# advimman/lama

Hardware: AMD Instinct MI355X
Metric: inpainted images/sec at 512x512 big-lama (higher is better)
Workload: dtype f32 (3-term f16 split on the 16-bit MFMA, fp32 accumulate, fp32 activations); 1 GPU; big-lama FFCResNetGenerator 512x512 batch=8/GPU fp32 (BASELINE configs[1]), mask-compose + generator + blend + u8, random-init weights; global_batch=8, resolution=512, parallelism=dp1, hip_graph=True, precision=f16x3, split_batch=1, full=False

## Files before the change

include/lama_hip.h:

```cpp
#ifndef LAMA_HIP_H
#define LAMA_HIP_H
#include <stddef.h>
#include <stdint.h>

#ifdef __cplusplus
extern "C" {
#endif

#define LAMA_HIP_VERSION 112

#define LAMA_OK 0
#define LAMA_ERR_BAD_ARG (-1)
#define LAMA_ERR_UNSUPPORTED (-2)
#define LAMA_ERR_WORKSPACE (-3)

#define LAMA_ACT_NONE 0
#define LAMA_ACT_RELU 1
#define LAMA_ACT_SIGMOID 2
#define LAMA_ACT_TANH 3

#define LAMA_PAD_ZERO 0
#define LAMA_PAD_REFLECT 1

#define LAMA_PREC_F32 0
// ... 116 lines not shown
    int32_t up_mg[4];
    int32_t* head_list;
    int32_t* head_count;
    int32_t* up_list[4];
    int32_t* up_count[4];
} lama_tail_lists;
size_t lama_tail_lists_workspace_bytes(int32_t batch, int32_t H, int32_t W, const lama_tail_lists* lists);
int lama_tail_lists_build(void* stream, const lama_tensor* mask, int32_t batch, const lama_tail_lists* lists, void* workspace, size_t workspace_bytes);
int lama_conv2d_list_fwd(void* stream, const lama_conv2d_args* args, const int32_t* list, const int32_t* count, int32_t head_rs);
int32_t lama_conv2d_list_supported(const lama_conv2d_args* args, int32_t head_rs);

#define LAMA_CONV_FAMILY_F32 0
#define LAMA_CONV_FAMILY_GEMM1X1_WK 1
#define LAMA_CONV_FAMILY_GEMM1X1_W4 2
#define LAMA_CONV_FAMILY_GEMM1X1_WS 3
#define LAMA_CONV_FAMILY_CONV_WR 4
#define LAMA_CONV_FAMILY_CONVT2 5
#define LAMA_CONV_FAMILY_STEM7 6
#define LAMA_CONV_FAMILY_HEAD7 7
#define LAMA_CONV_FAMILY_LDS 8
#define LAMA_CONV_GEO_WR(wmv, kg, ksc1, twlog, s2, coop, roll, fuse1, xs, ys) \
    ((wmv) | (kg) << 4 | (ksc1) << 8 | (twlog) << 12 | (s2) << 16 | (coop) << 17 | (roll) << 18 | (fuse1) << 19 | (xs) << 20 | (ys) << 21)
int lama_conv2d_route_query(const lama_conv2d_args* args, int32_t head_rs, int32_t* family, int32_t* geometry);

int lama_affine_act_fwd(void* stream, const lama_tensor* x, const float* scale, const float* shift, int32_t act,
                        const lama_tensor* y, int32_t batch);
int lama_reflect_pad_fwd(void* stream, const lama_tensor* x, int32_t pad, const lama_tensor* y, int32_t batch);

int lama_act_bwd(void* stream, const lama_tensor* g, const lama_tensor* y, int32_t act, const lama_tensor* gout, int32_t batch);
int lama_add_fwd(void* stream, const lama_tensor* a, const lama_tensor* b, const lama_tensor* out, int32_t batch);
int lama_reflect_pad_bwd(void* stream, const lama_tensor* gp, const lama_tensor* addend, int32_t pad, const lama_tensor* g,
                         int32_t batch);
int lama_reflect_pad_bwd_fused(void* stream, const lama_tensor* gp, const lama_tensor* add1, const lama_tensor* add2, int32_t pad,
                               const lama_tensor* mask_y, int32_t act, const lama_tensor* g, const lama_tensor* gm, int32_t batch,
                               const float* ring);
size_t lama_dgrad_ring_bytes(int32_t batch, int32_t cout, int32_t H, int32_t W);
int lama_dgrad_ring_fwd(void* stream, const lama_tensor* g, const float* w_ring, int32_t cout, float* ring, int32_t batch);
int lama_gauss5_fwd(void* stream, const lama_tensor* x, const lama_tensor* y, int32_t batch);
int lama_gauss5_bwd(void* stream, const lama_tensor* gy, const lama_tensor* gx, int32_t batch);
int lama_bilinear_fwd(void* stream, const lama_tensor* x, const lama_tensor* y, int32_t batch);
int lama_bilinear_bwd(void* stream, const lama_tensor* gy, const lama_tensor* gx, int32_t batch);
int lama_threshold_fwd(void* stream, const lama_tensor* x, float thr, const lama_tensor* y, int32_t batch);
int lama_erode_fwd(void* stream, const lama_tensor* x, const float* se, int32_t kh, int32_t kw, float max_val, const lama_tensor* y,
                   int32_t batch);
int lama_l1_masked_fwd(void* stream, const lama_tensor* pred, const lama_tensor* target, const lama_tensor* mask, float thr,
                       int32_t select_ge, double* accum, int32_t batch);
// ... 70 lines not shown
```

lama_amd/_lib.py:

```python
from __future__ import annotations

import ctypes as C
import os
from typing import Optional

import torch

ACT_NONE, ACT_RELU, ACT_SIGMOID, ACT_TANH = 0, 1, 2, 3
PAD_ZERO, PAD_REFLECT = 0, 1
PREC_F32, PREC_BF16X3, PREC_F16X3, PREC_F16 = 0, 1, 2, 3
CONV_COOPERATIVE = 1
CONV_DEFER_OUT = 2
CONV_SIBLINGS_SHIFT = 8
DT_F32, DT_F16, DT_SPLIT16 = 0, 1, 2
(CONV_FAM_F32, CONV_FAM_GEMM1X1_WK, CONV_FAM_GEMM1X1_W4, CONV_FAM_GEMM1X1_WS, CONV_FAM_CONV_WR, CONV_FAM_CONVT2, CONV_FAM_STEM7, CONV_FAM_HEAD7,
 CONV_FAM_LDS) = range(9)


def conv_geo_wr(wmv, kg, ksc1, twlog, s2=0, coop=0, roll=0, fuse1=0, xs=0, ys=0) -> int:
    return wmv | kg << 4 | ksc1 << 8 | twlog << 12 | s2 << 16 | coop << 17 | roll << 18 | fuse1 << 19 | xs << 20 | ys << 21


def conv_geo_lds(bm, bn, mode=0, trf=0) -> int:
    return bm | bn << 8 | mode << 20 | trf << 22
POOL_MAX, POOL_AVG_EXCLUDE_PAD = 0, 1
ABI_VERSION = 112
PREC_NAMES = {'f32': PREC_F32, 'bf16x3': PREC_BF16X3, 'f16x3': PREC_F16X3, 'f16': PREC_F16}

_DEFAULT = os.path.join(os.path.dirname(os.path.abspath(__file__)), 'lib', 'liblama_hip.so')


class LamaError(RuntimeError):

    def __init__(self, msg: str = '', code=None):
        super().__init__(msg)
        self.code = code


class LamaRangeError(LamaError):
# ... 79 lines not shown
    def __init__(self, path: Optional[str] = None, host_emulated: bool = False):
        self.host_emulated = host_emulated
        path = path or _DEFAULT
        if not os.path.exists(path):
            raise LamaError(f'{path} not found: build it with `python -m lama_amd.build` '
                            f'(hipcc --offload-arch=gfx950); lama_amd has no fallback path')
        self.path = path
        L = self._l = C.CDLL(path)
        i32, i64, vp, sz = C.c_int32, C.c_int64, C.c_void_p, C.c_size_t
        T = C.POINTER(Tensor4)
        L.lama_version.restype = C.c_int
        L.lama_error_string.restype = C.c_char_p
        L.lama_error_string.argtypes = [C.c_int]
        L.lama_conv2d_packed_weight_bytes.restype = i64
        L.lama_conv2d_packed_weight_bytes.argtypes = [i32] * 7
        L.lama_conv2d_pack_weight.restype = C.c_int
        L.lama_conv2d_pack_weight.argtypes = [vp, vp, vp, i32, i32, i32, i32, i32, i32, i32, vp]
        L.lama_conv2d_fwd.restype = C.c_int
        L.lama_conv2d_fwd.argtypes = [vp, C.POINTER(Conv2dArgs)]
        L.lama_conv2d_list_fwd.restype, L.lama_conv2d_list_fwd.argtypes = C.c_int, [vp, C.POINTER(Conv2dArgs), vp, vp, i32]
        L.lama_conv2d_list_supported.restype, L.lama_conv2d_list_supported.argtypes = i32, [C.POINTER(Conv2dArgs), i32]
        L.lama_conv2d_route_query.restype = C.c_int
        L.lama_conv2d_route_query.argtypes = [C.POINTER(Conv2dArgs), i32, C.POINTER(C.c_int32), C.POINTER(C.c_int32)]
        L.lama_tail_lists_workspace_bytes.restype, L.lama_tail_lists_workspace_bytes.argtypes = sz, [i32, i32, i32, C.POINTER(TailLists)]
        L.lama_tail_lists_build.restype, L.lama_tail_lists_build.argtypes = C.c_int, [vp, T, i32, C.POINTER(TailLists), vp, sz]
        L.lama_rfft2_fwd.restype = C.c_int
        L.lama_rfft2_fwd.argtypes = [vp, T, T, i32, vp, sz]
        L.lama_irfft2_fwd.restype = C.c_int
        L.lama_irfft2_fwd.argtypes = [vp, T, T, T, i32, vp, sz]
        L.lama_winograd_out_fwd.restype = C.c_int
        L.lama_winograd_out_fwd.argtypes = [vp, C.POINTER(Conv2dArgs), vp, sz]
        L.lama_rfft2_winograd_out_fwd.restype = C.c_int
        L.lama_rfft2_winograd_out_fwd.argtypes = [vp, T, T, i32, vp, sz, C.POINTER(Conv2dArgs), vp, sz]
        L.lama_rfft2_masked_fwd.restype = C.c_int
        L.lama_rfft2_masked_fwd.argtypes = [vp, T, T, T, i32, vp, sz]
        L.lama_irfft2_masked_fwd.restype = C.c_int
        L.lama_irfft2_masked_fwd.argtypes = [vp, T, T, T, T, i32, vp, sz]
        L.lama_fft_workspace_bytes.restype = sz
        L.lama_fft_workspace_bytes.argtypes = [i32] * 4
        L.lama_fft_route_query.restype = C.c_int
        L.lama_fft_route_query.argtypes = [T, T, T, T, i32, i32, vp, sz, C.POINTER(C.c_int32), C.POINTER(C.c_int32)]
        L.lama_fourier_unit_workspace_bytes.restype = sz
        L.lama_fourier_unit_workspace_bytes.argtypes = [i32] * 4
        L.lama_fourier_unit_fwd.restype = C.c_int
        L.lama_fourier_unit_fwd.argtypes = [vp, T, vp, vp, T, i32, i32, i32, vp, sz, vp]
        L.lama_fourier_unit_winograd_out_fwd.restype = C.c_int
# ... 94 lines not shown
            cout, cin, kh, kw = w.shape
        nbytes = self._l.lama_conv2d_packed_weight_bytes(cout, cin, kh, kw, stride, int(transposed), precision)
        if nbytes <= 0:
            raise LamaError(f'unsupported conv geometry {tuple(w.shape)} stride={stride} transposed={transposed}')
        if precision in (PREC_F16X3, PREC_F16) and w.numel():
            ws = w if scale is None else w * (scale.float().view(1, -1, 1, 1) if transposed else scale.float().view(-1, 1, 1, 1))
            amax = float(ws.abs().max())
            if not amax <= F16_MAX:
                raise LamaRangeError(f'folded conv weight |w| max {amax:.3g} exceeds the fp16 split range ({F16_MAX}); use bf16x3 or f32')
        dst = torch.empty(nbytes // 4, dtype=torch.float32, device=w.device)
        sc = None if scale is None else scale.contiguous().float()
        self.check(self._l.lama_conv2d_pack_weight(self.stream_of(w), w.data_ptr(), None if sc is None else sc.data_ptr(),
                                                   cout, cin, kh, kw, stride, int(transposed), precision, dst.data_ptr()),
                   'lama_conv2d_pack_weight')
        if w.is_cuda:
            torch.cuda.current_stream(w.device).synchronize()
        return dst

    def conv2d(self, x: Tensor4, w_packed: torch.Tensor, y: Tensor4, batch: int, k: int, stride: int = 1, pad: int = 0,
               pad_mode: int = PAD_REFLECT, transposed: bool = False, bias: Optional[torch.Tensor] = None,
               act: int = ACT_NONE, resid: Optional[Tensor4] = None, x2: Optional[Tensor4] = None,
               w2_packed: Optional[torch.Tensor] = None, precision: int = PREC_F32, stream: int = 0,
               range_flag: Optional[torch.Tensor] = None, fuse1: Optional[tuple] = None, cooperative: bool = False, siblings_log2: int = 0,
               tile_list: Optional[tuple] = None, query: bool = False, route: bool = False):
        a = Conv2dArgs()
        a.x, a.w_packed = x, w_packed.data_ptr()
        a.kh = a.kw = k
        a.stride, a.pad, a.pad_mode, a.transposed = stride, pad, pad_mode, int(transposed)
        if x2 is not None:
            a.x2, a.w2_packed = x2, w2_packed.data_ptr()
        a.bias = None if bias is None else bias.data_ptr()
        a.act = act
        if resid is not None:
            a.resid = resid
        a.y, a.batch, a.precision = y, batch, precision
        a.range_flag = None if range_flag is None else range_flag.data_ptr()
        if fuse1 is not None:
            a.fuse1_w, a.fuse1_bias, a.fuse1_y = fuse1[0].data_ptr(), fuse1[1].data_ptr(), fuse1[2]
        a.flags = (CONV_COOPERATIVE if cooperative else 0) | (int(siblings_log2) << CONV_SIBLINGS_SHIFT)
        if route:
            fam, geo = C.c_int32(-1), C.c_int32(-1)
            rc = self._l.lama_conv2d_route_query(C.byref(a), -1 if tile_list is None else int(tile_list[2]), C.byref(fam), C.byref(geo))
            return (int(rc), fam.value, geo.value) if rc == 0 else (int(rc), None, None)
        if tile_list is not None:
            lst, cnt, head_rs = tile_list
            if query:
                return self._l.lama_conv2d_list_supported(C.byref(a), int(head_rs)) == 1
            self.check(self._l.lama_conv2d_list_fwd(stream, C.byref(a), lst.data_ptr(), cnt.data_ptr(), int(head_rs)), 'lama_conv2d_list_fwd')
            return None
        self.check(self._l.lama_conv2d_fwd(stream, C.byref(a)), 'lama_conv2d_fwd')

    def tail_lists_alloc(self, batch: int, H: int, W: int, head_rs: int, up_mg, device) -> dict:
        n_up = len(up_mg)
        if n_up > 4 or H % (1 << n_up) or W % (1 << n_up) or head_rs < 8 or head_rs % 8:
            raise LamaError(f'tail lists: {n_up} upsamplings of a {H} x {W} plane, head_rs {head_rs}')

        def pair(n):
            return torch.zeros(n, dtype=torch.int32, device=device), torch.zeros(1, dtype=torch.int32, device=device)

        cd = lambda a, b: (a + b - 1) // b
        head = pair(batch * cd(W, 26) * cd(H, head_rs))
        up = [pair(batch * cd(H >> (i + 1), 4) * cd(W >> (i + 1), 32) * int(up_mg[i])) for i in range(n_up)]
        a = TailLists()
        a.n_up, a.head_rs = n_up, head_rs
        a.head_list, a.head_count = head[0].data_ptr(), head[1].data_ptr()
        for i in range(n_up):
# ... 492 lines not shown
```

lama_amd/csrc/conv_mfma.hip:

```cpp
#include "common.h"

typedef float f32x16 __attribute__((ext_vector_type(16)));

#define CONV_BN 128
#define CONV_MAX_TAPS 49

struct ConvSeg {
    const float* x;
    long long bstride;
    int C, H, W;
    const float* w;
    int stride, pad_mode;
    int dy0, dx0;
    int PH, PW;
    int tapoff[CONV_MAX_TAPS];
};

struct ConvParams {
    ConvSeg s1, s2;
    const float* bias;
    const float* resid;
    long long resid_bstride;
    float* y;
    long long y_bstride;
// ... 658 lines not shown
        p.tiles_y = lama_ceil_div(p.GH, CONV_BN >> twlog);
        int T2 = 0, BKC2 = 0;
        if (has2) {
            T2 = 1; BKC2 = pl2.BKC[0];
            if (!fill_seg(&p.s2, a->x2, (const float*)a->w2_packed, pl2, 0, 1, LAMA_PAD_ZERO, twlog, BKC2 * CONV_BN / LAMA_NTHREADS, false))
                return LAMA_ERR_UNSUPPORTED;
        }
        int rc = launch_conv((hipStream_t)stream, p, pl.T[cls], pl.BKC[cls], T2, BKC2, pl.BM, query != nullptr);
        if (rc != LAMA_OK) return rc;
    }
    return LAMA_OK;
}

extern "C" int lama_conv2d_fwd(void* stream, const lama_conv2d_args* a) { return conv2d_impl(stream, a, nullptr); }

extern "C" int lama_conv2d_list_fwd(void* stream, const lama_conv2d_args* a, const int32_t* list, const int32_t* count, int32_t head_rs) {
    if (!list || !count) return LAMA_ERR_BAD_ARG;
    const LamaTileList tl = {list, count, head_rs};
    return conv2d_impl(stream, a, &tl);
}
extern "C" int lama_conv2d_route_query(const lama_conv2d_args* a, int32_t head_rs, int32_t* family, int32_t* geometry) {
    if (!family || !geometry) return LAMA_ERR_BAD_ARG;
    const LamaTileList tl = {nullptr, nullptr, head_rs};
    int32_t q[2] = {0, 0};
    const int rc = conv2d_impl(nullptr, a, head_rs < 0 ? nullptr : &tl, q);
    if (rc == LAMA_OK) { *family = q[0]; *geometry = q[1]; }
    return rc;
}
extern "C" int32_t lama_conv2d_list_supported(const lama_conv2d_args* a, int32_t head_rs) {
    int32_t family, geometry;
    return lama_conv2d_route_query(a, head_rs < 0 ? 0 : head_rs, &family, &geometry) == LAMA_OK ? 1 : 0;
}
```

lama_amd/csrc/conv_split3.inc:

```
#include "common.h"
#include <stdlib.h>

typedef float f32x16 __attribute__((ext_vector_type(16)));
typedef float f32x2 __attribute__((ext_vector_type(2)));
#ifndef CB_HALF
#define CB_HALF 0
#endif
#ifndef CB_HF_W2
#define CB_HF_W2 1
#endif
#if CB_F16
typedef _Float16 cb_half_t;
#define CB_MFMA __builtin_amdgcn_mfma_f32_32x32x16_f16
#if CB_HALF
#define CB_NAME(x) x##_f16
#else
#define CB_NAME(x) x##_f16x3
#endif
#else
typedef __bf16 cb_half_t;
#define CB_MFMA __builtin_amdgcn_mfma_f32_32x32x16_bf16
#define CB_NAME(x) x##_bf16x3
#endif
typedef cb_half_t bf16x2 __attribute__((ext_vector_type(2)));
// ... 897 lines not shown
        pp.kw = kw;
        pp.transposed = transposed;
        for (int t = 0; t < pl.T[cls]; ++t) { pp.tap_ky[t] = pl.ky[cls][t]; pp.tap_kx[t] = pl.kx[cls][t]; }
        long long total = pl.cls_bytes[cls] / 32;
        int grid = (int)((total + 255) / 256);
        if (grid > 4096) grid = 4096;
        hipLaunchKernelGGL(CB_NAME(conv_pack_kernel), dim3(grid), dim3(256), 0, stream, pp);
        LAMA_CHECK_LAUNCH();
    }
    return LAMA_OK;
}

int CB_NAME(lama_cb_conv2d_fwd)(hipStream_t stream, const lama_conv2d_args* a, int Ho, int Wo, const LamaTileList* tl, int32_t* query) {
    CbPlan pl, pl2;
    if (!cb_make_plan(a->y.C, a->x.C, a->kh, a->kw, a->stride, a->pad, a->transposed, &pl)) return LAMA_ERR_UNSUPPORTED;
    const bool has2 = a->x2.ptr != nullptr;
    if (has2 && (!cb_make_plan(a->y.C, a->x2.C, 1, 1, 1, 0, 0, &pl2) || pl.mode)) return LAMA_ERR_UNSUPPORTED;
    int io = (a->x.dtype == LAMA_DT_F16 ? 1 : 0) | (a->y.dtype == LAMA_DT_F16 ? 2 : 0) | ((has2 && a->x2.dtype == LAMA_DT_F16) ? CB_IO_X2H : 0);
    if ((io != CB_IO_F32) != (CB_HALF != 0)) return LAMA_ERR_UNSUPPORTED;
    io |= (a->x.dtype == LAMA_DT_SPLIT16 ? CB_IO_XS : 0) | (a->y.dtype == LAMA_DT_SPLIT16 ? CB_IO_YS : 0);
    const CbPlan* p2 = has2 ? &pl2 : nullptr;
    CbRoute r;
    const int rc = cb_route(a, pl, p2, Ho, Wo, io, tl, &r);
    if (query && rc == LAMA_OK) { query[0] = r.family; query[1] = cb_route_geometry(r); }
    if (query || rc != LAMA_OK) return rc;
    const long long HW = (long long)Ho * Wo;
    switch (r.family) {
        case CB_FAM_WK: return wk_launch(stream, a, pl, HW, r);
        case CB_FAM_W4: return w4_launch(stream, a, pl, HW, r);
        case CB_FAM_WS: return ws_launch(stream, a, pl, HW, r);
        case CB_FAM_WR: return wr_launch(stream, a, pl, p2, Ho, Wo, r);
        case CB_FAM_CT: return ct_launch(stream, a, pl, tl, r);
        case CB_FAM_STEM: return stem_launch(stream, a, pl, Ho, Wo, r);
        case CB_FAM_HEAD: return head_launch(stream, a, pl, Ho, Wo, tl, r);
        case CB_FAM_LDS: {
            CbParams p;
            lds_fill(&p, a, pl, p2, Ho, Wo, r);
            return cb_launch(stream, p, pl.T[0], has2 ? 1 : 0, r.BM, r.maxu, r.trf, r.mode, io, r.grid, r.shmem);
        }
    }
    return CB_ERR_ROUTE;
}

#if !CB_HALF
int CB_NAME(lama_cb_mdconv_fwd)(hipStream_t stream, const lama_conv2d_args* a, int groups, int min_dilation) {
    const int cout = a->y.C, cin = a->x.C, H = a->x.H, W = a->x.W;
    const int dmax = min_dilation << (groups - 1);
// ... 236 lines not shown
```

lama_amd/csrc/conv_wreg_dev.inc:

```

template <int T, int KSC, int WMV, int KG>
struct CwShape {
    static_assert((T == 9 && (KSC == 2 || (KSC == 1 && KG == 1))) || (T == 1 && KSC == 4),
                  "3x3 over 32-channel chunks (16-channel chunks in the 4 x 1 geometry) or 1x1 over 64-channel chunks");
    static_assert(KG == 1 || KG == 2, "K-groups");
    static constexpr int THREADS = 64 * WMV * KG;
    static constexpr int NKG = T * KSC / KG;
    static constexpr int WPS = WMV * KG / 4;
    static constexpr int PFD = (T == 1 && KG == 2) ? 2 : 1;
#ifndef LAMA_CW_RING9
#define LAMA_CW_RING9 0
#endif
    static constexpr int RING = (T == 9) ? ((LAMA_CW_RING9 && KG == 2 && WPS <= 2) ? 9 : ((KSC == 2 && WMV == 4 && KG == 1) ? 6 : 3)) : ((WPS >= 3) ? 2 : 4);
    static constexpr bool BDB = WPS <= 2;
    static constexpr int NOCT = 2 * KSC;
    static_assert((PFD * NKG) % RING == 0, "ring slot must be a compile-time function of the unrolled position");
};

struct CwFrag {
    bf16x8 bh[4], bl[4];
};

template <int T, int KSC, int WMV, int KG, int ABL = 0, int SCH = 2, bool HF = false, bool HI = HF, bool ROLL = false, int NU = 2, bool XS = false>
__device__ __forceinline__ void cw_segment(const CbSeg& s, int F, int b, int gy0, int gx0, int TWlog, char* pbuf0, int pbytes,
// ... 362 lines not shown
    const int tiy = tile % p.tiles_y;
    const int b = tile / p.tiles_y;
    const int TW = 1 << p.TWlog, TH = 128 >> p.TWlog;
    const int gy0 = tiy * TH, gx0 = tix * TW;
    const int tid = threadIdx.x, lane = tid & 63, wave = LAMA_WAVE_UNIFORM(tid >> 6);
    const int kg = wave / WMV, wm = wave % WMV;
    const int F = mt * WMV + wm;
    const int Fc = F < p.s1.mft ? F : p.s1.mft - 1;

    long long* trace = nullptr;
    if constexpr (ABL & 64) {
        trace = p.trace + (long long)blockIdx.x * 32;
        if (threadIdx.x == 0) trace[0] = LAMA_CLOCK();
    }
    f32x16 acc[4];
#pragma unroll
    for (int j = 0; j < 4; ++j)
#pragma unroll
        for (int r = 0; r < 16; ++r) acc[j][r] = 0.0f;

    unsigned rw = 0;
    const int Fw = (ABL & 256) ? Fc % 6 : Fc;
    cw_segment<T1, KSC1, WMV, KG, (ABL & 255), SCH, HF, HI1, ROLL && T1 == 9, NU, XS>(p.s1, Fw, b, gy0, gx0, p.TWlog, lama_smem, p.pbytes, acc, rw, trace);
    if constexpr (T2 > 0) cw_segment<T2, KSC2, WMV, KG, (ABL & 65), SCH, HF, HI2>(p.s2, Fw, b, gy0, gx0, p.TWlog, lama_smem, p.pbytes, acc, rw, (ABL & 64) ? trace + 7 : nullptr);
    cb_range_report(rw, p.range_flag);

    const long long plane = (long long)p.Ho * p.Wo;
    const int khalf4 = 4 * (lane >> 5);
    const int kplane = khalf4 * (int)plane;
    auto row_u = [&](int r) { return F * 32 + (r & 3) + 8 * (r >> 2); };
    float bv[16];
#pragma unroll
    for (int r = 0; r < 16; ++r) bv[r] = p.bias ? p.bias[row_u(r) + khalf4 < p.M ? row_u(r) + khalf4 : p.M - 1] : 0.0f;
    constexpr int NRV = (WMV * KG / 4 >= 3) ? 1 : 2;
    float rv[NRV][16];
    auto frag_off = [&](int j, bool& pv) {
        const int n = j * 32 + (lane & 31);
        const int gy = gy0 + (n >> p.TWlog), gx = gx0 + (n & (TW - 1));
        pv = gy < p.GH && gx < p.GW;
        return (gy < p.GH ? gy : p.GH - 1) * p.Wo + (gx < p.GW ? gx : p.GW - 1);
    };
    auto load_resid = [&](int j, int slot) {
        bool pv;
        const int po = frag_off(j, pv);
#pragma unroll
        for (int r = 0; r < 16; ++r) {
            const int mu = row_u(r), muc = mu < p.M ? mu : p.M - 1;
// ... 191 lines not shown
```

lama_amd/csrc/conv_wreg_host.inc:

```

#define G4_SUP 2
#ifndef GK_DEFAULT_MODE
#define GK_DEFAULT_MODE 1
#endif

enum CbFamily {
    CB_FAM_WK = LAMA_CONV_FAMILY_GEMM1X1_WK, CB_FAM_W4 = LAMA_CONV_FAMILY_GEMM1X1_W4, CB_FAM_WS = LAMA_CONV_FAMILY_GEMM1X1_WS,
    CB_FAM_WR = LAMA_CONV_FAMILY_CONV_WR, CB_FAM_CT = LAMA_CONV_FAMILY_CONVT2, CB_FAM_STEM = LAMA_CONV_FAMILY_STEM7,
    CB_FAM_HEAD = LAMA_CONV_FAMILY_HEAD7, CB_FAM_LDS = LAMA_CONV_FAMILY_LDS
};

struct CbRoute {
    int family;
    int io;
    bool list;
    int WMV, KG, KSC1, twlog;
    bool s2, coop, roll, fuse1;
    int NH, nch;
    bool rs;
    int BM, BN, mode, maxu;
    bool trf;
    int grid, ntiles, nslots, aux, seg_rows;
    size_t shmem;
};

int cb_route_geometry(const CbRoute& r) {
    const int xs = (r.io & CB_IO_XS) ? 1 : 0, ys = (r.io & CB_IO_YS) ? 1 : 0;
    switch (r.family) {
        case CB_FAM_WK: return r.aux;
        case CB_FAM_W4: return r.nch << 4 | (int)r.rs << 8;
        case CB_FAM_WS: return r.NH | r.nch << 4 | (int)r.rs << 8;
        case CB_FAM_WR: return LAMA_CONV_GEO_WR(r.WMV, r.KG, r.KSC1, r.twlog, (int)r.s2, (int)r.coop, (int)r.roll, (int)r.fuse1, xs, ys);
        case CB_FAM_CT: case CB_FAM_HEAD: return r.list ? 1 : 0;
        case CB_FAM_STEM: return ys << 21;
        case CB_FAM_LDS: return r.BM | r.BN << 8 | r.mode << 20 | (int)r.trf << 22;
    }
    return 0;
}

static inline bool cb_span_fits(long long bstride, int batch, long long C, long long HW, long long limit) {
// ... 263 lines not shown

bool ct_route(const lama_conv2d_args* a, const CbPlan& pl, int Ho, int Wo, int io, CbRoute* r) {
#if CB_HALF
    (void)a; (void)pl; (void)Ho; (void)Wo; (void)io; (void)r;
    return false;
#else
    const int mode = lama_env_int("LAMA_CT", 1);
    if (mode == 0 || !a->transposed || pl.nseg != 5 || pl.mode != 0 || io != CB_IO_F32 || a->resid.ptr || a->fuse1_w) return false;
    const int C = a->x.C, H = a->x.H, W = a->x.W, M = pl.rows;
    if (C % 32 != 0 || M % 64 != 0 || H < 1 || W < 1 || Ho != 2 * H || Wo != 2 * W) return false;
    if (!cb_span_fits(0, 1, C, (long long)H * W, 1ll << 31)) return false;
    CtParams p;
    if (!ct_fill(&p, a, pl) || p.T[0] != 4 || p.T[3] != 1 || p.T[1] != 2 || p.T[2] != 2) return false;
    bool table_ok = true;
    for (int q = 0; q < 9; ++q) table_ok = table_ok && p.off[c2_cls(q)][c2_tap(q)] == c2_dy(q) * CT_PWS + c2_dx(q);
    for (int c = 0; c < 4; ++c) table_ok = table_ok && p.py[c] == (c < 2 ? 1 : 0) && p.px[c] == ((c == 0 || c == 2) ? 1 : 0);
    if (!table_ok || !cb_act_linear(a)) return false;
    if ((a->y.batch_stride % 4) != 0 || ((uintptr_t)a->y.ptr & 15) != 0) return false;
    const long long tiles = (long long)a->batch * p.tiles_x * p.tiles_y * p.MG;
    if (tiles >= (1ll << 30)) return false;
    long long grid = tiles < 512 ? tiles : 512;
    { const int cap = lama_env_int("LAMA_CT_GRID", 0); if (cap > 0 && grid > cap) grid = cap; }
    r->grid = (int)grid;
    return true;
#endif
}

bool stem_route(const lama_conv2d_args* a, const CbPlan& pl, int Ho, int Wo, int io, CbRoute* r) {
#if CB_HALF
    if (io != CB_IO_F32_F16) return false;
#else
    if (io != CB_IO_F32 && !(io == CB_IO_YS && pl.rows % 8 == 0)) return false;
#endif
    static const int mode = lama_env_int("LAMA_STEM_WS", 1);
    if (mode == 0 || pl.mode != 1 || pl.mft != 2 || a->transposed || a->stride != 1 || a->pad != 3 || a->pad_mode != LAMA_PAD_REFLECT ||
        a->resid.ptr || a->x.H < 4 || a->x.W < 4)
        return false;
    const long long HW = (long long)Ho * Wo;
    if (!cb_span_fits(0, 1, a->x.C, HW, 1ll << 31) || !cb_span_fits(0, 1, 64, HW, 1ll << 31)) return false;
    const long long cols = (long long)a->batch * lama_ceil_div(Wo, 32);
    if (mode != 2 && cols * Ho < 4096) return false;
    long long ns = cols >= 1024 ? 1 : lama_ceil_div64(1024, cols);
    if (ns > Ho) ns = Ho;
    r->seg_rows = (int)lama_ceil_div64(Ho, ns);
    const long long nseg = cols * lama_ceil_div(Ho, r->seg_rows);
    if (nseg >= (1ll << 31)) return false;
// ... 303 lines not shown
    if (r.KG == 2) CW_GO(CW_LOCAL_42, CW_F32, 5);
    CW_GO(CW_LOCAL_41, CW_F32, 5);
#endif
    return CB_ERR_ROUTE;
}

int wr_launch(hipStream_t st, const lama_conv2d_args* a, const CbPlan& pl, const CbPlan* pl2, int Ho, int Wo, const CbRoute& r) {
    if (r.grid <= 0) return LAMA_OK;
    CbParams p;
    wr_fill(&p, a, pl, pl2, Ho, Wo, r);
    const int T1 = pl.T[0];
#if defined(LAMA_PROFILING) && !CB_HALF
    if (CB_F16) {
        static const int abl = lama_env_int("LAMA_CW_ABLATE", 0);
        static const int sch = lama_env_int("LAMA_CW_SCHED", 2);
        static const unsigned long long tr = lama_env_u64("LAMA_CW_TRACE");
        if (T1 == 9 && !pl2 && r.WMV == 4 && !r.s2) {
#define CW_ABL(v) if (abl == v && p.TWlog == 5) CW_GO(CW_LOCAL_42, v, 2, false, false, false, false, true);
            CW_ABL(1) CW_ABL(2) CW_ABL(4) CW_ABL(3) CW_ABL(7) CW_ABL(8) CW_ABL(16) CW_ABL(32) CW_ABL(128) CW_ABL(132) CW_ABL(135)
#undef CW_ABL
            if (sch == 0) CW_GO(CW_LOCAL_42, 0, 0);
            if (sch == 1) CW_GO(CW_LOCAL_42, 0, 1);
        }
        if (pl2 && r.WMV == 12 && T1 == 9 && r.io == CB_IO_F32 && (abl == 1 || abl == 256)) {
            if (r.fuse1) { if (abl == 1) CW_GO(CW_GLOBAL_12, 1, 2, false, false, false, false, false, 2, true); else CW_GO(CW_GLOBAL_12, 256, 2, false, false, false, false, false, 2, true); }
            if (abl == 1) CW_GO(CW_GLOBAL_12, 1);
            CW_GO(CW_GLOBAL_12, 256);
        }
        if (tr && pl2 && r.WMV == 12) { p.trace = reinterpret_cast<long long*>(tr); CW_GO(CW_GLOBAL_12, 64); }
        if (tr && !pl2 && !r.s2) {
            p.trace = reinterpret_cast<long long*>(tr);
            if (T1 == 9 && p.TWlog == 5) CW_GO(CW_LOCAL_42, 64, 2, false, false, false, false, true);
            if (T1 == 9) CW_GO(CW_LOCAL_42, 64);
            if (r.WMV == 12) CW_GO(CW_1X1_12, 64);
            if (r.WMV == 6) CW_GO(CW_1X1_62, 64);
            CW_GO(CW_1X1_42, 64);
        }
    }
#endif
    if (r.s2) return wr_launch_s2(st, p, r);
#if !CB_HALF
    if (r.coop) { if (r.roll) CW_GO(CW_LOCAL_COOP, CW_F32_ROLL, 4); else CW_GO(CW_LOCAL_COOP, CW_F32, 4); }
#endif
    if (T1 == 9 && !pl2) return r.KG == 1 ? wr_launch_io<CW_LOCAL_41>(st, p, r) : wr_launch_io<CW_LOCAL_42>(st, p, r);
#if !CB_HALF
    if (r.fuse1) CW_GO(CW_GLOBAL_12, CW_F32, 2, true);
#endif
    if (T1 == 9) return r.WMV == 12 ? wr_launch_io<CW_GLOBAL_12>(st, p, r) : wr_launch_io<CW_GLOBAL_42>(st, p, r);
    if (r.WMV == 12) return wr_launch_io<CW_1X1_12>(st, p, r);
    if (r.WMV == 6) return wr_launch_io<CW_1X1_62>(st, p, r);
    return wr_launch_io<CW_1X1_42>(st, p, r);
}
#undef CW_GO

int ct_launch(hipStream_t stream, const lama_conv2d_args* a, const CbPlan& pl, const LamaTileList* tl, const CbRoute& r) {
#if CB_HALF
    (void)stream; (void)a; (void)pl; (void)tl; (void)r;
    return CB_ERR_ROUTE;
#else
    if (r.grid <= 0) return LAMA_OK;
    CtParams p;
    ct_fill(&p, a, pl);
    { static const int abl = lama_env_int("LAMA_CT_ABLATE", 0); p.abl = abl; }
    if (tl) {
        p.list = tl->list; p.count = tl->count;
        hipLaunchKernelGGL(CB_NAME(convt2_kernel)<true>, dim3(r.grid), dim3(C2_THREADS), C2_LDS_BYTES, stream, p);
    } else
        hipLaunchKernelGGL(CB_NAME(convt2_kernel)<false>, dim3(r.grid), dim3(C2_THREADS), C2_LDS_BYTES, stream, p);
    LAMA_CHECK_LAUNCH();
    return LAMA_OK;
#endif
}

int stem_launch(hipStream_t stream, const lama_conv2d_args* a, const CbPlan& pl, int Ho, int Wo, const CbRoute& r) {
    StemParams p;
    memset(&p, 0, sizeof(p));
    p.x = (const float*)a->x.ptr;
    p.x_bstride = a->x.batch_stride;
    p.C = a->x.C; p.H = Ho; p.W = Wo;
    p.w = (const char*)a->w_packed + pl.woff[0];
    p.mft = pl.mft;
    p.bias = a->bias;
    p.y = (float*)a->y.ptr;
    p.y_bstride = a->y.batch_stride;
    p.M = pl.rows;
    p.B = a->batch;
    p.act = a->act;
    p.range_flag = a->range_flag;
    p.tx = lama_ceil_div(Wo, 32);
    p.rs = r.seg_rows;
// ... 44 lines not shown
```

lama_amd/csrc/convt_dev.inc:

```

struct CtParams {
    const float* x;
    long long x_bstride;
    int C, H, W;
    const char* w[4];
    int T[4];
    int off[4][4];
    int py[4], px[4];
    int mft;
    const float* bias;
    float* y;
    long long y_bstride;
    int M, B, act;
    int tiles_x, tiles_y, MG;
    unsigned* range_flag;
    int abl;
    const int* list;
    const int* count;
};

#define CT_PWS 34
#define CT_NPIX (5 * CT_PWS)

#define C2_THREADS 256
#ifndef C2_KG
#define C2_KG 1
#endif
#ifndef C2_AR
#define C2_AR 3
#endif
#define C2_NU ((2 * C2_KG * 165 + C2_THREADS - 1) / C2_THREADS)
#define C2_PLANES (2 * C2_KG * CT_NPIX * 16)
#define C2_PBUF (2 * C2_PLANES)
#define C2_LDS_BYTES (2 * C2_PBUF + 32)
#ifndef C2_ABL
#define C2_ABL 0
#endif

constexpr int c2_cls(int q) { constexpr int t[9] = {0, 1, 2, 3, 0, 1, 0, 2, 0}; return t[q]; }
constexpr int c2_tap(int q) { constexpr int t[9] = {3, 1, 1, 0, 1, 0, 2, 0, 0}; return t[q]; }
constexpr int c2_dy(int q) { constexpr int t[9] = {0, 0, 0, 0, 1, 1, 0, 0, 1}; return t[q]; }
constexpr int c2_dx(int q) { constexpr int t[9] = {0, 0, 0, 0, 0, 0, 1, 1, 1}; return t[q]; }

template <bool LIST = false>
__global__ __launch_bounds__(C2_THREADS, 2) void CB_NAME(convt2_kernel)(CtParams p) {
    static_assert((C2_AR == 3 || C2_AR == 6) && (C2_KG == 1 || C2_KG == 2), "ring slot = compile-time function of (k-group parity, position)");
    constexpr int KG = C2_KG, AR = C2_AR, NU = C2_NU;
    const int tid = threadIdx.x, lane = tid & 63, wave = LAMA_WAVE_UNIFORM(tid >> 6);
    const int f = wave & 1, pp = wave >> 1;
    const int khalf = lane >> 5, l31 = lane & 31;
    const int HW = p.H * p.W;
    char* const smem = lama_smem;
    const int L0 = lama_xcd_remap(blockIdx.x, gridDim.x), G = gridDim.x;
    const int ndense = p.B * p.tiles_y * p.tiles_x * p.MG;
    int ntiles = ndense;
    if constexpr (LIST) { const int n = p.count[0]; ntiles = n < ntiles ? (n > 0 ? n : 0) : ntiles; }
    const int ntl = L0 < ntiles ? (ntiles - L0 + G - 1) / G : 0;
    const int ngr = p.C / 16, nch = ngr / KG, nseq = ntl * nch;
    auto tile_of = [&](int tl, int& mg, int& b, int& gy0, int& gx0) {
        int t0 = L0 + tl * G;
        if constexpr (LIST) { t0 = p.list[t0]; t0 = t0 < 0 ? 0 : (t0 >= ndense ? ndense - 1 : t0); }
        mg = t0 % p.MG;
        t0 /= p.MG;
        const int tx = t0 % p.tiles_x;
        t0 /= p.tiles_x;
        gy0 = (t0 % p.tiles_y) * 4;
        gx0 = tx * 32;
        b = t0 / p.tiles_y;
    };
    int uinf[NU];
#pragma unroll
    for (int i = 0; i < NU; ++i) {
        const int u = tid + i * C2_THREADS;
        uinf[i] = -1;
        if (u < 2 * KG * 165) {
            const int o = u / 165, pq = u - o * 165, ry = pq / 33;
            uinf[i] = (o << 16) | (ry << 8) | (pq - ry * 33);
        }
    }
    float preg[NU][8];
    unsigned rw = 0;
    lama_buf_t xres;
    int vo[NU];
    auto unit_addr = [&](int sq) {
        const bool live = sq < nseq;
        const int tl = live ? sq / nch : 0, c = live ? sq - tl * nch : 0;
        int mg, b, gy0, gx0;
        tile_of(tl, mg, b, gy0, gx0);
        xres = LAMA_BUF_RSRC(reinterpret_cast<const char*>(p.x) + (long long)b * p.x_bstride * 4 + (long long)c * 16 * KG * HW * 4,
                             live ? (long long)(p.C - c * 16 * KG) * HW * 4 : 0ll);
#pragma unroll
        for (int i = 0; i < NU; ++i) {
            const int iy = gy0 + ((uinf[i] >> 8) & 255), ix = gx0 + (uinf[i] & 255);
            vo[i] = (uinf[i] >= 0 && iy < p.H && ix < p.W) ? ((uinf[i] >> 16) * 8 * HW + iy * p.W + ix) * 4 : 0x7ffffff0;
        }
    };
    auto load_part = [&](int e) {
        if constexpr (C2_ABL & 4) return;
#pragma unroll
        for (int i = 0; i < NU; ++i) preg[i][e] = __builtin_bit_cast(float, LAMA_BUF_LOAD_B32(xres, vo[i], e * HW * 4));
    };
    auto load_units = [&](int sq) {
        unit_addr(sq);
#pragma unroll
        for (int e = 0; e < 8; ++e) load_part(e);
    };
    u32x4 sh, sl;
    auto split_unit = [&](int i) {
        unsigned hh[4], ll[4];
#pragma unroll
        for (int e = 0; e < 4; ++e) cb_split2(preg[i][2 * e], preg[i][2 * e + 1], hh[e], ll[e], rw);
        sh = u32x4{hh[0], hh[1], hh[2], hh[3]};
        sl = u32x4{ll[0], ll[1], ll[2], ll[3]};
    };
    auto store_unit = [&](char* buf, int i) {
        if constexpr (C2_ABL & 64) { LAMA_KEEP_LIVE(sh); LAMA_KEEP_LIVE(sl); return; }
        char* d = uinf[i] >= 0 ? buf + ((uinf[i] >> 16) * CT_NPIX + ((uinf[i] >> 8) & 255) * CT_PWS + (uinf[i] & 255)) * 16 : smem + 2 * C2_PBUF;
        *reinterpret_cast<u32x4*>(d) = sh;
        *reinterpret_cast<u32x4*>(d + (uinf[i] >= 0 ? C2_PLANES : 16)) = sl;
    };
    auto write_units = [&](char* buf) {
#pragma unroll
        for (int i = 0; i < NU; ++i) { split_unit(i); store_unit(buf, i); }
    };
    const lama_buf_t wres0 = LAMA_BUF_RSRC(p.w[0], (long long)(p.C / 16) * 4 * p.mft * 2048);
    const lama_buf_t wres1 = LAMA_BUF_RSRC(p.w[1], (long long)(p.C / 16) * 2 * p.mft * 2048);
    const lama_buf_t wres2 = LAMA_BUF_RSRC(p.w[2], (long long)(p.C / 16) * 2 * p.mft * 2048);
    const lama_buf_t wres3 = LAMA_BUF_RSRC(p.w[3], (long long)(p.C / 16) * 1 * p.mft * 2048);
    bf16x8 ah[AR], al[AR];
    auto load_a = [&](auto q_tag, int g, int F, auto slot_tag) {
        constexpr int q = decltype(q_tag)::value, S = decltype(slot_tag)::value;
        constexpr int cls = c2_cls(q), T = cls == 0 ? 4 : (cls == 3 ? 1 : 2);
        const int so = ((g * T + c2_tap(q)) * p.mft + F) * 2048;
#define C2_LOAD_A(wr)                                                                      \
    do {                                                                                   \
        ah[S] = __builtin_bit_cast(bf16x8, LAMA_BUF_LOAD_B128(wr, lane * 16, so));         \
        al[S] = __builtin_bit_cast(bf16x8, LAMA_BUF_LOAD_B128(wr, lane * 16 + 1024, so));  \
    } while (0)
        if constexpr (cls == 0) C2_LOAD_A(wres0);
        else if constexpr (cls == 1) C2_LOAD_A(wres1);
        else if constexpr (cls == 2) C2_LOAD_A(wres2);
        else C2_LOAD_A(wres3);
#undef C2_LOAD_A
    };
    const int boff = (khalf * CT_NPIX + 2 * pp * CT_PWS + l31) * 16;
    bf16x8 bh[3][2], bl[3][2];
// ... 149 lines not shown
```

Measured before the change: 860.2 images/s.

## Add wide 128-bit input staging path for transposed-conv kernel

Adds a wide-staging variant of the convt2 kernel in which each thread loads four consecutive pixels per channel with 128-bit buffer loads, replacing one 32-bit load per pixel per channel. The thread-to-unit mapping is redesigned (192 group slots plus 20 column units) and the split/store to LDS is rearranged to match. It is enabled by default when W is a multiple of 4 and the input is 16-byte aligned, and a query API reports which staging form was chosen. It also adds extra ablation dispatch variants for the wreg conv. The aim is fewer global load instructions in the upsampling convs; the risk lies in the more complex index mapping and the uneven split of threads into units.

```diff
diff --git a/include/lama_hip.h b/include/lama_hip.h
--- a/include/lama_hip.h
+++ b/include/lama_hip.h
@@ -162,6 +162,9 @@
 #define LAMA_CONV_GEO_WR(wmv, kg, ksc1, twlog, s2, coop, roll, fuse1, xs, ys) \
     ((wmv) | (kg) << 4 | (ksc1) << 8 | (twlog) << 12 | (s2) << 16 | (coop) << 17 | (roll) << 18 | (fuse1) << 19 | (xs) << 20 | (ys) << 21)
 int lama_conv2d_route_query(const lama_conv2d_args* args, int32_t head_rs, int32_t* family, int32_t* geometry);
+#define LAMA_CONV_STAGING_PIXEL 0
+#define LAMA_CONV_STAGING_WIDE 1
+int lama_conv2d_staging_query(const lama_conv2d_args* args, int32_t head_rs, int32_t* staging);
 
 int lama_affine_act_fwd(void* stream, const lama_tensor* x, const float* scale, const float* shift, int32_t act,
                         const lama_tensor* y, int32_t batch);
diff --git a/lama_amd/_lib.py b/lama_amd/_lib.py
--- a/lama_amd/_lib.py
+++ b/lama_amd/_lib.py
@@ -15,6 +15,9 @@
 DT_F32, DT_F16, DT_SPLIT16 = 0, 1, 2
 (CONV_FAM_F32, CONV_FAM_GEMM1X1_WK, CONV_FAM_GEMM1X1_W4, CONV_FAM_GEMM1X1_WS, CONV_FAM_CONV_WR, CONV_FAM_CONVT2, CONV_FAM_STEM7, CONV_FAM_HEAD7,
  CONV_FAM_LDS) = range(9)
+
+
+CONV_STAGING_PIXEL, CONV_STAGING_WIDE = 0, 1
 
 
 def conv_geo_wr(wmv, kg, ksc1, twlog, s2=0, coop=0, roll=0, fuse1=0, xs=0, ys=0) -> int:
@@ -140,6 +143,8 @@
         L.lama_conv2d_list_supported.restype, L.lama_conv2d_list_supported.argtypes = i32, [C.POINTER(Conv2dArgs), i32]
         L.lama_conv2d_route_query.restype = C.c_int
         L.lama_conv2d_route_query.argtypes = [C.POINTER(Conv2dArgs), i32, C.POINTER(C.c_int32), C.POINTER(C.c_int32)]
+        L.lama_conv2d_staging_query.restype = C.c_int
+        L.lama_conv2d_staging_query.argtypes = [C.POINTER(Conv2dArgs), i32, C.POINTER(C.c_int32)]
         L.lama_tail_lists_workspace_bytes.restype, L.lama_tail_lists_workspace_bytes.argtypes = sz, [i32, i32, i32, C.POINTER(TailLists)]
         L.lama_tail_lists_build.restype, L.lama_tail_lists_build.argtypes = C.c_int, [vp, T, i32, C.POINTER(TailLists), vp, sz]
         L.lama_rfft2_fwd.restype = C.c_int
@@ -280,7 +285,7 @@
                act: int = ACT_NONE, resid: Optional[Tensor4] = None, x2: Optional[Tensor4] = None,
                w2_packed: Optional[torch.Tensor] = None, precision: int = PREC_F32, stream: int = 0,
                range_flag: Optional[torch.Tensor] = None, fuse1: Optional[tuple] = None, cooperative: bool = False, siblings_log2: int = 0,
-               tile_list: Optional[tuple] = None, query: bool = False, route: bool = False):
+               tile_list: Optional[tuple] = None, query: bool = False, route: bool = False, staging: bool = False):
         a = Conv2dArgs()
         a.x, a.w_packed = x, w_packed.data_ptr()
         a.kh = a.kw = k
@@ -300,6 +305,10 @@
             fam, geo = C.c_int32(-1), C.c_int32(-1)
             rc = self._l.lama_conv2d_route_query(C.byref(a), -1 if tile_list is None else int(tile_list[2]), C.byref(fam), C.byref(geo))
             return (int(rc), fam.value, geo.value) if rc == 0 else (int(rc), None, None)
+        if staging:
+            form = C.c_int32(-1)
+            rc = self._l.lama_conv2d_staging_query(C.byref(a), -1 if tile_list is None else int(tile_list[2]), C.byref(form))
+            return (int(rc), form.value if rc == 0 else None)
         if tile_list is not None:
             lst, cnt, head_rs = tile_list
             if query:
diff --git a/lama_amd/csrc/conv_mfma.hip b/lama_amd/csrc/conv_mfma.hip
--- a/lama_amd/csrc/conv_mfma.hip
+++ b/lama_amd/csrc/conv_mfma.hip
@@ -704,11 +704,19 @@
 extern "C" int lama_conv2d_route_query(const lama_conv2d_args* a, int32_t head_rs, int32_t* family, int32_t* geometry) {
     if (!family || !geometry) return LAMA_ERR_BAD_ARG;
     const LamaTileList tl = {nullptr, nullptr, head_rs};
-    int32_t q[2] = {0, 0};
+    int32_t q[3] = {0, 0, 0};
     const int rc = conv2d_impl(nullptr, a, head_rs < 0 ? nullptr : &tl, q);
     if (rc == LAMA_OK) { *family = q[0]; *geometry = q[1]; }
     return rc;
 }
+extern "C" int lama_conv2d_staging_query(const lama_conv2d_args* a, int32_t head_rs, int32_t* staging) {
+    if (!staging) return LAMA_ERR_BAD_ARG;
+    const LamaTileList tl = {nullptr, nullptr, head_rs};
+    int32_t q[3] = {0, 0, LAMA_CONV_STAGING_PIXEL};
+    const int rc = conv2d_impl(nullptr, a, head_rs < 0 ? nullptr : &tl, q);
+    if (rc == LAMA_OK) *staging = q[2];
+    return rc;
+}
 extern "C" int32_t lama_conv2d_list_supported(const lama_conv2d_args* a, int32_t head_rs) {
     int32_t family, geometry;
     return lama_conv2d_route_query(a, head_rs < 0 ? 0 : head_rs, &family, &geometry) == LAMA_OK ? 1 : 0;
diff --git a/lama_amd/csrc/conv_split3.inc b/lama_amd/csrc/conv_split3.inc
--- a/lama_amd/csrc/conv_split3.inc
+++ b/lama_amd/csrc/conv_split3.inc
@@ -943,7 +943,7 @@
     const CbPlan* p2 = has2 ? &pl2 : nullptr;
     CbRoute r;
     const int rc = cb_route(a, pl, p2, Ho, Wo, io, tl, &r);
-    if (query && rc == LAMA_OK) { query[0] = r.family; query[1] = cb_route_geometry(r); }
+    if (query && rc == LAMA_OK) { query[0] = r.family; query[1] = cb_route_geometry(r); query[2] = r.wide ? LAMA_CONV_STAGING_WIDE : LAMA_CONV_STAGING_PIXEL; }
     if (query || rc != LAMA_OK) return rc;
     const long long HW = (long long)Ho * Wo;
     switch (r.family) {
diff --git a/lama_amd/csrc/conv_wreg_dev.inc b/lama_amd/csrc/conv_wreg_dev.inc
--- a/lama_amd/csrc/conv_wreg_dev.inc
+++ b/lama_amd/csrc/conv_wreg_dev.inc
@@ -408,7 +408,7 @@
     unsigned rw = 0;
     const int Fw = (ABL & 256) ? Fc % 6 : Fc;
     cw_segment<T1, KSC1, WMV, KG, (ABL & 255), SCH, HF, HI1, ROLL && T1 == 9, NU, XS>(p.s1, Fw, b, gy0, gx0, p.TWlog, lama_smem, p.pbytes, acc, rw, trace);
-    if constexpr (T2 > 0) cw_segment<T2, KSC2, WMV, KG, (ABL & 65), SCH, HF, HI2>(p.s2, Fw, b, gy0, gx0, p.TWlog, lama_smem, p.pbytes, acc, rw, (ABL & 64) ? trace + 7 : nullptr);
+    if constexpr (T2 > 0) cw_segment<T2, KSC2, WMV, KG, (ABL & 117), SCH, HF, HI2>(p.s2, Fw, b, gy0, gx0, p.TWlog, lama_smem, p.pbytes, acc, rw, (ABL & 64) ? trace + 7 : nullptr);
     cb_range_report(rw, p.range_flag);
 
     const long long plane = (long long)p.Ho * p.Wo;
diff --git a/lama_amd/csrc/conv_wreg_host.inc b/lama_amd/csrc/conv_wreg_host.inc
--- a/lama_amd/csrc/conv_wreg_host.inc
+++ b/lama_amd/csrc/conv_wreg_host.inc
@@ -16,6 +16,7 @@
     bool list;
     int WMV, KG, KSC1, twlog;
     bool s2, coop, roll, fuse1;
+    bool wide;
     int NH, nch;
     bool rs;
     int BM, BN, mode, maxu;
@@ -325,6 +326,8 @@
     long long grid = tiles < 512 ? tiles : 512;
     { const int cap = lama_env_int("LAMA_CT_GRID", 0); if (cap > 0 && grid > cap) grid = cap; }
     r->grid = (int)grid;
+    static const int wide = lama_env_int("LAMA_CT_WIDE", 1);
+    r->wide = wide != 0 && W % 4 == 0 && ((uintptr_t)a->x.ptr & 15) == 0 && a->x.batch_stride % 4 == 0;
     return true;
 #endif
 }
@@ -674,6 +677,11 @@
             if (sch == 0) CW_GO(CW_LOCAL_42, 0, 0);
             if (sch == 1) CW_GO(CW_LOCAL_42, 0, 1);
         }
+        if (pl2 && r.WMV == 12 && T1 == 9 && r.io == CB_IO_F32 && r.fuse1 && (abl == 4 || abl == 16 || abl == 32)) {
+            if (abl == 4) CW_GO(CW_GLOBAL_12, 4, 2, false, false, false, false, false, 2, true);
+            if (abl == 16) CW_GO(CW_GLOBAL_12, 16, 2, false, false, false, false, false, 2, true);
+            CW_GO(CW_GLOBAL_12, 32, 2, false, false, false, false, false, 2, true);
+        }
         if (pl2 && r.WMV == 12 && T1 == 9 && r.io == CB_IO_F32 && (abl == 1 || abl == 256)) {
             if (r.fuse1) { if (abl == 1) CW_GO(CW_GLOBAL_12, 1, 2, false, false, false, false, false, 2, true); else CW_GO(CW_GLOBAL_12, 256, 2, false, false, false, false, false, 2, true); }
             if (abl == 1) CW_GO(CW_GLOBAL_12, 1);
@@ -716,8 +724,11 @@
     { static const int abl = lama_env_int("LAMA_CT_ABLATE", 0); p.abl = abl; }
     if (tl) {
         p.list = tl->list; p.count = tl->count;
-        hipLaunchKernelGGL(CB_NAME(convt2_kernel)<true>, dim3(r.grid), dim3(C2_THREADS), C2_LDS_BYTES, stream, p);
-    } else
+        if (r.wide) hipLaunchKernelGGL((CB_NAME(convt2_kernel)<true, true>), dim3(r.grid), dim3(C2_THREADS), C2_LDS_BYTES, stream, p);
+        else hipLaunchKernelGGL(CB_NAME(convt2_kernel)<true>, dim3(r.grid), dim3(C2_THREADS), C2_LDS_BYTES, stream, p);
+    } else if (r.wide)
+        hipLaunchKernelGGL((CB_NAME(convt2_kernel)<false, true>), dim3(r.grid), dim3(C2_THREADS), C2_LDS_BYTES, stream, p);
+    else
         hipLaunchKernelGGL(CB_NAME(convt2_kernel)<false>, dim3(r.grid), dim3(C2_THREADS), C2_LDS_BYTES, stream, p);
     LAMA_CHECK_LAUNCH();
     return LAMA_OK;
diff --git a/lama_amd/csrc/convt_dev.inc b/lama_amd/csrc/convt_dev.inc
--- a/lama_amd/csrc/convt_dev.inc
+++ b/lama_amd/csrc/convt_dev.inc
@@ -42,10 +42,11 @@
 constexpr int c2_dy(int q) { constexpr int t[9] = {0, 0, 0, 0, 1, 1, 0, 0, 1}; return t[q]; }
 constexpr int c2_dx(int q) { constexpr int t[9] = {0, 0, 0, 0, 0, 0, 1, 1, 1}; return t[q]; }
 
-template <bool LIST = false>
+template <bool LIST = false, bool WS = false>
 __global__ __launch_bounds__(C2_THREADS, 2) void CB_NAME(convt2_kernel)(CtParams p) {
     static_assert((C2_AR == 3 || C2_AR == 6) && (C2_KG == 1 || C2_KG == 2), "ring slot = compile-time function of (k-group parity, position)");
-    constexpr int KG = C2_KG, AR = C2_AR, NU = C2_NU;
+    static_assert(!WS || C2_KG == 1, "wide staging: one 16-channel k-group per chunk (192 group slots + 20 column units on 256 threads)");
+    constexpr int KG = C2_KG, AR = C2_AR, NU = WS ? 1 : C2_NU, NPR = WS ? 16 : 8;
     const int tid = threadIdx.x, lane = tid & 63, wave = LAMA_WAVE_UNIFORM(tid >> 6);
     const int f = wave & 1, pp = wave >> 1;
     const int khalf = lane >> 5, l31 = lane & 31;
@@ -73,12 +74,21 @@
     for (int i = 0; i < NU; ++i) {
         const int u = tid + i * C2_THREADS;
         uinf[i] = -1;
-        if (u < 2 * KG * 165) {
+        if constexpr (WS) {
+            if (u < 192) {
+                const int g = (u & 3) | ((u >> 4) & 1) << 2, h = (u >> 3) & 1, rest = u >> 5;
+                const int ry = ((u >> 2) & 1) + 2 * (rest % 3), o = rest / 3;
+                if (ry < 5) uinf[i] = ((2 * o + h) << 16) | (ry << 8) | (4 * g);
+            } else if (u < 212) {
+                const int t = u - 192;
+                uinf[i] = (1 << 24) | ((t & 3) << 16) | ((t >> 2) << 8) | 32;
+            }
+        } else if (u < 2 * KG * 165) {
             const int o = u / 165, pq = u - o * 165, ry = pq / 33;
             uinf[i] = (o << 16) | (ry << 8) | (pq - ry * 33);
         }
     }
-    float preg[NU][8];
+    float preg[NU][NPR];
     unsigned rw = 0;
     lama_buf_t xres;
     int vo[NU];
@@ -92,11 +102,23 @@
 #pragma unroll
         for (int i = 0; i < NU; ++i) {
             const int iy = gy0 + ((uinf[i] >> 8) & 255), ix = gx0 + (uinf[i] & 255);
-            vo[i] = (uinf[i] >= 0 && iy < p.H && ix < p.W) ? ((uinf[i] >> 16) * 8 * HW + iy * p.W + ix) * 4 : 0x7ffffff0;
+            if constexpr (WS) vo[i] = (uinf[i] >= 0 && iy < p.H && ix < p.W) ? (((uinf[i] >> 16) & 255) * 4 * HW + iy * p.W + ix) * 4 : 0x7ffffff0;
+            else vo[i] = (uinf[i] >= 0 && iy < p.H && ix < p.W) ? ((uinf[i] >> 16) * 8 * HW + iy * p.W + ix) * 4 : 0x7ffffff0;
         }
     };
     auto load_part = [&](int e) {
         if constexpr (C2_ABL & 4) return;
+        if constexpr (WS) {
+            if (e < 4) {
+                const u32x4 v = __builtin_bit_cast(u32x4, LAMA_BUF_LOAD_B128(xres, vo[0], e * HW * 4));
+#pragma unroll
+                for (int j = 0; j < 4; ++j) {
+                    const unsigned vj = v[j];
+                    preg[0][4 * e + j] = __builtin_bit_cast(float, vj);
+                }
+            }
+            return;
+        }
 #pragma unroll
         for (int i = 0; i < NU; ++i) preg[i][e] = __builtin_bit_cast(float, LAMA_BUF_LOAD_B32(xres, vo[i], e * HW * 4));
     };
@@ -107,6 +129,17 @@
     };
     u32x4 sh, sl;
     auto split_unit = [&](int i) {
+        if constexpr (WS) {
+            unsigned hh[4], ll[4];
+#pragma unroll
+            for (int k = 0; k < 2; ++k) {
+                cb_split2(preg[0][2 * i + k], preg[0][4 + 2 * i + k], hh[2 * k], ll[2 * k], rw);
+                cb_split2(preg[0][8 + 2 * i + k], preg[0][12 + 2 * i + k], hh[2 * k + 1], ll[2 * k + 1], rw);
+            }
+            sh = u32x4{hh[0], hh[1], hh[2], hh[3]};
+            sl = u32x4{ll[0], ll[1], ll[2], ll[3]};
+            return;
+        }
         unsigned hh[4], ll[4];
 #pragma unroll
         for (int e = 0; e < 4; ++e) cb_split2(preg[i][2 * e], preg[i][2 * e + 1], hh[e], ll[e], rw);
@@ -115,13 +148,25 @@
     };
     auto store_unit = [&](char* buf, int i) {
         if constexpr (C2_ABL & 64) { LAMA_KEEP_LIVE(sh); LAMA_KEEP_LIVE(sl); return; }
+        if constexpr (WS) {
+            const int hq = (uinf[0] >> 16) & 255;
+            char* const d0 = buf + ((hq >> 1) * CT_NPIX + ((uinf[0] >> 8) & 255) * CT_PWS + (uinf[0] & 255)) * 16 + 8 * (hq & 1);
+#pragma unroll
+            for (int k = 0; k < 2; ++k) {
+                const bool real = uinf[0] >= 0 && ((uinf[0] >> 24) == 0 || 2 * i + k == 0);
+                char* d = real ? d0 + (2 * i + k) * 16 : smem + 2 * C2_PBUF;
+                *reinterpret_cast<u32x2*>(d) = u32x2{sh[2 * k], sh[2 * k + 1]};
+                *reinterpret_cast<u32x2*>(d + (real ? C2_PLANES : 16)) = u32x2{sl[2 * k], sl[2 * k + 1]};
+            }
+            return;
+        }
         char* d = uinf[i] >= 0 ? buf + ((uinf[i] >> 16) * CT_NPIX + ((uinf[i] >> 8) & 255) * CT_PWS + (uinf[i] & 255)) * 16 : smem + 2 * C2_PBUF;
         *reinterpret_cast<u32x4*>(d) = sh;
         *reinterpret_cast<u32x4*>(d + (uinf[i] >= 0 ? C2_PLANES : 16)) = sl;
     };
     auto write_units = [&](char* buf) {
 #pragma unroll
-        for (int i = 0; i < NU; ++i) { split_unit(i); store_unit(buf, i); }
+        for (int i = 0; i < (WS ? 2 : NU); ++i) { split_unit(i); store_unit(buf, i); }
     };
     const lama_buf_t wres0 = LAMA_BUF_RSRC(p.w[0], (long long)(p.C / 16) * 4 * p.mft * 2048);
     const lama_buf_t wres1 = LAMA_BUF_RSRC(p.w[1], (long long)(p.C / 16) * 2 * p.mft * 2048);
```

Result: no change. 859.8 images/s (-0.0%).
